# nianticlabs/relpose-gnn

Hardware: AMD Instinct MI355X
Metric: graphs/sec (8-node fully-connected, 224x224) (higher is better)
Workload: dtype f32; 1 GPU; BASELINE.json configs[1]: batch=32 8-node fully-connected graphs per GPU, 224x224 RGB, fp32, ResNet34 + GNN (D=2048, gnn_recursion=2, droprate=0, eval), random-init weights; nodes_per_graph=8, edges_per_graph=56, streams_per_gpu=2, loaded_library=relpose-gnn_amd/lib/librelpose_gnn_hip.so@26afda1856ea

## Files before the change

relpose-gnn_amd/csrc/winograd.hip:

```cpp
#include "rpg_common.h"

typedef float f32x16 __attribute__((ext_vector_type(16)));

namespace {

constexpr int NT = 256;
constexpr int BK = 16, LD = BK;
constexpr int P = 6;
constexpr int BMT = 64, BN = 64;
constexpr int A_FLOATS = P * BMT * LD, B_FLOATS = P * BN * LD;
constexpr int LDS_BYTES = (A_FLOATS + B_FLOATS) * (int)sizeof(float);

struct Epi {
    const float* scale;
    const float* shift;
    const float* residual;
    float* out;
    int relu;
};

__device__ __forceinline__ float4 f4zero() { return make_float4(0.f, 0.f, 0.f, 0.f); }
__device__ __forceinline__ float4 lin(float a, const float4& x, float b, const float4& y) {
    return make_float4(a * x.x + b * y.x, a * x.y + b * y.y, a * x.z + b * y.z, a * x.w + b * y.w);
}
__device__ __forceinline__ float4 add(const float4& x, const float4& y) {
    return make_float4(x.x + y.x, x.y + y.y, x.z + y.z, x.w + y.w);
}
__device__ __forceinline__ float4 sub(const float4& x, const float4& y) {
    return make_float4(x.x - y.x, x.y - y.y, x.z - y.z, x.w - y.w);
}

typedef unsigned int u32x4 __attribute__((ext_vector_type(4)));
typedef float f32x2 __attribute__((ext_vector_type(2)));
__device__ __forceinline__ void wino43_epilogue(const f32x16 (&acc)[P], float* slab, int lane, int mw0, int nw0, int M,
                                                int Tw, int W, int Cout, const Epi& ep) {
    constexpr int EP = 32 + 4;
    constexpr unsigned OOB = 0x80000000u;
    const int c4 = lane & 7, pr = lane >> 3;
    const int nb = nw0 + 4 * c4;
    const bool n_ok = nb < Cout;
    float4 sc = make_float4(1.f, 1.f, 1.f, 1.f), sh = f4zero();
    if (n_ok && ep.scale) sc = *reinterpret_cast<const float4*>(ep.scale + nb);
    if (n_ok && ep.shift) sh = *reinterpret_cast<const float4*>(ep.shift + nb);

    const int t_first = mw0 / Tw;
    const size_t row0 = (size_t)t_first * W * Cout;
    const __amdgpu_buffer_rsrc_t ro = __builtin_amdgcn_make_buffer_rsrc(ep.out + row0, 0, 0x7fffffff, 0x00020000);
    const __amdgpu_buffer_rsrc_t rr = __builtin_amdgcn_make_buffer_rsrc(
        const_cast<float*>(ep.residual ? ep.residual + row0 : ep.out + row0), 0, 0x7fffffff, 0x00020000);
    const int step_t = 4 / Tw, step_tw = 4 % Tw;
    int mt = mw0 + (pr >> 1);
    int trel = mt / Tw - t_first, tw = mt % Tw;
    unsigned voff[2][8];
#pragma unroll
    for (int it = 0; it < 8; ++it) {
        const int wo = 4 * tw + (pr & 1);
        const bool ok = n_ok && mt < M;
        const unsigned o = 4u * (unsigned)((trel * W + wo) * Cout + nb);
        voff[0][it] = ok && wo < W ? o : OOB;
        voff[1][it] = ok && wo + 2 < W ? o + 8u * (unsigned)Cout : OOB;
        mt += 4;
        trel += step_t;
        tw += step_tw;
        if (tw >= Tw) { tw -= Tw; ++trel; }
    }
    float4 rs[2][8];
    if (ep.residual) {
#pragma unroll
        for (int half = 0; half < 2; ++half)
#pragma unroll
            for (int it = 0; it < 8; ++it)
                rs[half][it] = __builtin_bit_cast(float4, __builtin_amdgcn_raw_buffer_load_b128(rr, voff[half][it], 0, 0));
    } else {
#pragma unroll
        for (int half = 0; half < 2; ++half)
#pragma unroll
            for (int it = 0; it < 8; ++it) rs[half][it] = f4zero();
    }
    const bool relu_on = ep.relu;
    f32x2 y[4][8];
#pragma unroll
    for (int q = 0; q < 8; ++q) {
        const int e = 2 * q;
        const f32x2 m0 = {acc[0][e], acc[0][e + 1]}, m1 = {acc[1][e], acc[1][e + 1]}, m2 = {acc[2][e], acc[2][e + 1]};
        const f32x2 m3 = {acc[3][e], acc[3][e + 1]}, m4 = {acc[4][e], acc[4][e + 1]}, m5 = {acc[5][e], acc[5][e + 1]};
        const f32x2 s12 = m1 + m2, d12 = m1 - m2, s34 = m3 + m4, d34 = m3 - m4;
        const f32x2 u = d34 + d34;
        y[0][q] = (m0 + s12) + s34;
        y[1][q] = d12 + u;
        y[2][q] = s12 + 4.f * s34;
        y[3][q] = (d12 + 4.f * u) + m5;
    }
#pragma unroll
    for (int half = 0; half < 2; ++half) {
#pragma unroll
        for (int q = 0; q < 8; ++q) {
            const int e = 2 * q;
            const int trow = (e & 3) + 8 * (e >> 2) + 4 * (lane >> 5);
            float* sp = slab + (2 * trow) * EP + (lane & 31);
            sp[0] = y[2 * half][q].x;
            sp[EP] = y[2 * half + 1][q].x;
            sp[2 * EP] = y[2 * half][q].y;
            sp[3 * EP] = y[2 * half + 1][q].y;
        }
        __builtin_amdgcn_wave_barrier();
#pragma unroll
        for (int it = 0; it < 8; ++it) {
            const int prow = pr + 8 * it;
            const float4 v = *reinterpret_cast<const float4*>(&slab[prow * EP + 4 * c4]);
            const f32x2 r0 = {rs[half][it].x, rs[half][it].y}, r1 = {rs[half][it].z, rs[half][it].w};
            f32x2 o0 = f32x2{v.x, v.y} * f32x2{sc.x, sc.y} + f32x2{sh.x, sh.y} + r0;
            f32x2 o1 = f32x2{v.z, v.w} * f32x2{sc.z, sc.w} + f32x2{sh.z, sh.w} + r1;
            const float4 yv = rpg::relu4_if(relu_on, make_float4(o0.x, o0.y, o1.x, o1.y));
            __builtin_amdgcn_raw_buffer_store_b128(__builtin_bit_cast(u32x4, yv), ro, voff[half][it], 0, 0);
        }
        __builtin_amdgcn_wave_barrier();
    }
}

template <bool RES, class Mid>
__device__ __forceinline__ void wino43_epilogue_lean_body(const f32x16 (&acc)[P], float* slab, int lane, int mw0, int nw0, int M,
                                                          int Tw, int W, int Cout, const Epi& ep, Mid mid) {
    constexpr int EP = 32 + 4;
    constexpr unsigned OOB = 0x80000000u;
    const int c4 = lane & 7, pr = lane >> 3;
    const int nb = nw0 + 4 * c4;
    const bool n_ok = nb < Cout;
    float4 sc = make_float4(1.f, 1.f, 1.f, 1.f), sh = f4zero();
    if (n_ok && ep.scale) sc = *reinterpret_cast<const float4*>(ep.scale + nb);
    if (n_ok && ep.shift) sh = *reinterpret_cast<const float4*>(ep.shift + nb);
    const int t_first = mw0 / Tw;
    const size_t row0 = (size_t)t_first * W * Cout;
    const __amdgpu_buffer_rsrc_t ro = __builtin_amdgcn_make_buffer_rsrc(ep.out + row0, 0, 0x7fffffff, 0x00020000);
    const __amdgpu_buffer_rsrc_t rr = __builtin_amdgcn_make_buffer_rsrc(
        const_cast<float*>(ep.residual ? ep.residual + row0 : ep.out + row0), 0, 0x7fffffff, 0x00020000);
    const int step_t = 4 / Tw, step_tw = 4 % Tw;
    int mt = mw0 + (pr >> 1);
    int trel = mt / Tw - t_first, tw = mt % Tw;
    unsigned voff[8], ok2 = 0;
#pragma unroll
    for (int it = 0; it < 8; ++it) {
// ... 232 lines not shown
        __syncthreads();
        float4 fa[2][2], fb[2][2];
        auto frag_one = [&](int g, int set, int i) {
            const int kb = (g / 3) * 8, xi = 2 * (g % 3) + (i >> 1);
            if (i & 1) fb[set][i >> 1] = *reinterpret_cast<const float4*>(&Bs[xi * BN * LD + (b_off ^ kb)]);
            else       fa[set][i >> 1] = *reinterpret_cast<const float4*>(&As[xi * BMT * LD + (a_off ^ kb)]);
        };
#pragma unroll
        for (int i = 0; i < 4; ++i) frag_one(0, 0, i);
        __builtin_amdgcn_sched_barrier(0);
#pragma unroll
        for (int g = 0; g < 6; ++g) {
            const int set = g & 1, x0 = 2 * (g % 3);
#pragma unroll
            for (int i = 0; i < 8; ++i) {
                const int j = i & 1, e = i >> 1;
                const float av = e == 0 ? fa[set][j].x : e == 1 ? fa[set][j].y : e == 2 ? fa[set][j].z : fa[set][j].w;
                const float bv = e == 0 ? fb[set][j].x : e == 1 ? fb[set][j].y : e == 2 ? fb[set][j].z : fb[set][j].w;
                acc[x0 + j] = __builtin_amdgcn_mfma_f32_32x32x2f32(av, bv, acc[x0 + j], 0, 0, 0);
                if (i < 4 && g + 1 < 6) frag_one(g + 1, set ^ 1, i);
                if (i >= 4 && i < 6) fetch_one(2 * g + (i - 4));
                __builtin_amdgcn_sched_barrier(0);
            }
        }
        fetch_next();
    }
    __syncthreads();

    const int ws = __builtin_amdgcn_readfirstlane(wave);
    wino43_epilogue(acc, lds + ws * (64 * 36), lane, m0 + (ws >> 1) * 32, n0 + (ws & 1) * 32, M, Tw, W, Cout, ep);
}

constexpr int NT8 = 512, BMT8 = 128;
constexpr int A8_FLOATS = P * BMT8 * LD, IMG8_FLOATS = A8_FLOATS + B_FLOATS;
constexpr int LDS8_BYTES = 2 * IMG8_FLOATS * (int)sizeof(float);

typedef float f32x2 __attribute__((ext_vector_type(2)));
struct F4 { f32x2 lo, hi; };
__device__ __forceinline__ F4 to_f4(const float4& v) { return F4{f32x2{v.x, v.y}, f32x2{v.z, v.w}}; }
__device__ __forceinline__ float4 to_float4(const F4& v) { return make_float4(v.lo.x, v.lo.y, v.hi.x, v.hi.y); }
#define RPG_PK_FMA(NAME, CONST)                                                                               \
    __device__ __forceinline__ f32x2 NAME(f32x2 x, f32x2 y) {                                                 \
        f32x2 r;                                                                                              \
        asm("v_pk_fma_f32 %0, %1, " CONST ", %2 op_sel_hi:[1,0,1]" : "=v"(r) : "v"(x), "v"(y));               \
        return r;                                                                                             \
    }
RPG_PK_FMA(pk_fma_p4, "4.0")
RPG_PK_FMA(pk_fma_m4, "-4.0")
RPG_PK_FMA(pk_fma_p2, "2.0")
RPG_PK_FMA(pk_fma_m2, "-2.0")
#undef RPG_PK_FMA
__device__ __forceinline__ f32x2 pk_add(f32x2 x, f32x2 y) {
    f32x2 r;
    asm("v_pk_add_f32 %0, %1, %2" : "=v"(r) : "v"(x), "v"(y));
    return r;
}
__device__ __forceinline__ f32x2 pk_sub(f32x2 x, f32x2 y) {
    f32x2 r;
    asm("v_pk_add_f32 %0, %1, %2 neg_lo:[0,1] neg_hi:[0,1]" : "=v"(r) : "v"(x), "v"(y));
    return r;
}
#define RPG_F4_OP(NAME, OP) \
    __device__ __forceinline__ F4 NAME(const F4& x, const F4& y) { return F4{OP(x.lo, y.lo), OP(x.hi, y.hi)}; }
RPG_F4_OP(fma4_p4, pk_fma_p4)
RPG_F4_OP(fma4_m4, pk_fma_m4)
RPG_F4_OP(fma4_p2, pk_fma_p2)
RPG_F4_OP(fma4_m2, pk_fma_m2)
RPG_F4_OP(add4, pk_add)
RPG_F4_OP(sub4, pk_sub)
#undef RPG_F4_OP

struct Split { int tile_base, parts, n_split; float* partial; unsigned* arrive; };

#ifdef RPG_WINO_TRACE
__device__ unsigned long long* g_wino_trace = nullptr;
#define RPG_TRACE(i)                                                                         \
    do {                                                                                     \
        if (g_wino_trace && threadIdx.x == 0) g_wino_trace[5 * blockIdx.x + (i)] = __builtin_readcyclecounter(); \
    } while (0)
#else
#define RPG_TRACE(i) do {} while (0)
#endif

__device__ __forceinline__ void wino43_finish_quad(const float4& s, const Epi& ep, int tile, int p, int c4, int M, int Tw, int W,
                                                   int Cout, int tiles_n) {
    const int m = (tile / tiles_n) * BMT8 + (p >> 2), nb = (tile % tiles_n) * BN + 4 * c4;
    if (m >= M || nb >= Cout) return;
    const int t = m / Tw, wo = 4 * (m - t * Tw) + (p & 3);
    if (wo >= W) return;
    const size_t o = ((size_t)t * W + wo) * Cout + nb;
    float4 sc = make_float4(1.f, 1.f, 1.f, 1.f), sh = f4zero(), rs = f4zero();
    if (ep.scale) sc = *reinterpret_cast<const float4*>(ep.scale + nb);
    if (ep.shift) sh = *reinterpret_cast<const float4*>(ep.shift + nb);
    if (ep.residual) rs = *reinterpret_cast<const float4*>(ep.residual + o);
    float4 y;
    y.x = s.x * sc.x + sh.x + rs.x; y.y = s.y * sc.y + sh.y + rs.y;
    y.z = s.z * sc.z + sh.z + rs.z; y.w = s.w * sc.w + sh.w + rs.w;
    if (ep.relu) y = rpg::relu4(y);
    *reinterpret_cast<float4*>(ep.out + o) = y;
}

__device__ __forceinline__ void wino43_combine_last(const Split& sp, int tt, const Epi& ep, int M, int Tw, int W, int Cout,
                                                    int tiles_n, int* flag) {
    if (!rpg::last_arriver(sp.arrive + tt, (unsigned)sp.parts, flag)) return;
    const __amdgpu_buffer_rsrc_t rs = rpg::agent_rsrc(sp.partial + (size_t)tt * sp.parts * (BMT8 * 4 * BN));
    constexpr unsigned SLAB_B = BMT8 * 4 * BN * 4;
    const int tile = sp.tile_base + tt;
    const int tid_c = threadIdx.x;
#pragma unroll 1
    for (int h = 0; h < 2; ++h) {
        const unsigned vo = 16u * (unsigned)(tid_c + h * 8 * NT8);
        float4 sum[8];
#pragma unroll
        for (int c = 0; c < 8; ++c) sum[c] = rpg::agent_load_f4(rs, vo + 16u * c * NT8, 0);
        for (int i = 1; i < sp.parts; ++i) {
            float4 v[8];
#pragma unroll
            for (int c = 0; c < 8; ++c) v[c] = rpg::agent_load_f4(rs, vo + 16u * c * NT8, (unsigned)i * SLAB_B);
#pragma unroll
            for (int c = 0; c < 8; ++c) { sum[c].x += v[c].x; sum[c].y += v[c].y; sum[c].z += v[c].z; sum[c].w += v[c].w; }
        }
#pragma unroll
        for (int c = 0; c < 8; ++c) {
            const int idx = tid_c + NT8 * (8 * h + c);
            wino43_finish_quad(sum[c], ep, tile, idx >> 4, idx & 15, M, Tw, W, Cout, tiles_n);
        }
    }
}

__global__ __launch_bounds__(NT8) void wino43_conv8_kernel(const float* __restrict__ x, const float* __restrict__ U, int H,
                                                          int W, int Cin, int Cout, int Tw, int M, Epi ep, int tiles_n,
                                                          Split sp) {
    extern __shared__ __attribute__((aligned(16))) float lds[];
#ifdef RPG_WINO_TRACE
    if (g_wino_trace && threadIdx.x == 0) g_wino_trace[5 * blockIdx.x] = __builtin_amdgcn_s_getreg(0xF804);
#endif
    RPG_TRACE(1);
    const int K = 3 * Cin;
    const int kpr = (Cin + BK - 1) / BK;
    int tile, kb = 0, nk = 3 * kpr;
    const bool is_split = (int)blockIdx.x < sp.n_split;
    if (is_split) {
        const int tt = blockIdx.x / sp.parts, part = blockIdx.x - tt * sp.parts;
        tile = sp.tile_base + tt;
        kb = 3 * (part * kpr / sp.parts);
        nk = 3 * ((part + 1) * kpr / sp.parts);
    } else {
        const int nwg = gridDim.x - sp.n_split, bid = blockIdx.x - sp.n_split;
        const int xcd = bid & 7, loc = bid >> 3, q = nwg >> 3, r8 = nwg & 7;
        tile = (xcd < r8 ? xcd * (q + 1) : r8 * (q + 1) + (xcd - r8) * q) + loc;
    }
    const int m0 = (tile / tiles_n) * BMT8;
    const int n0 = (tile % tiles_n) * BN;

    const int tid = threadIdx.x, lane = tid & 63, wave = tid >> 6;
    const int wm = wave >> 1, wn = wave & 1;
    const int row = tid >> 2, slot = tid & 3;
    const int brow = row & 63, bhalf = tid >> 8;

    const int n_first = (m0 / Tw) / H;
    const size_t img_floats = (size_t)H * W * Cin;
    const __amdgpu_buffer_rsrc_t ra = __builtin_amdgcn_make_buffer_rsrc(
        const_cast<float*>(x + n_first * img_floats) - (size_t)W * Cin, 0, 0x7fffffff, 0x00020000);
    const __amdgpu_buffer_rsrc_t rb = __builtin_amdgcn_make_buffer_rsrc(const_cast<float*>(U), 0, 0x7fffffff, 0x00020000);
    constexpr unsigned OOB = 0x80000000u;
    unsigned va[P], va3[3][P];
    unsigned rowbits = 0;
    {
        const int m = m0 + row;
        int img_off = 0, ho = 0, wi0 = -(1 << 24);
        if (m < M) {
            const int tw = m % Tw;
            const int t = m / Tw;
            ho = t % H;
            img_off = (t / H - n_first) * (int)img_floats;
            wi0 = 4 * tw - 1;
            rowbits = (ho > 0 ? 1u : 0u) | 2u | (ho < H - 1 ? 4u : 0u);
        }
#pragma unroll
        for (int j = 0; j < P; ++j) {
            const int wi = wi0 + j;
            va[j] = (unsigned)wi < (unsigned)W ? 4u * (unsigned)(img_off + (ho * W + wi) * Cin + 4 * slot) : OOB;
        }
    }
    const unsigned ustride_b = (unsigned)Cout * K * 4u;
    const unsigned vb = n0 + brow < Cout ? 4u * (unsigned)((n0 + brow) * K + 4 * slot) + 3u * bhalf * ustride_b : OOB;
    unsigned vb_eff;
    int f_kt = kb, f_c0 = (kb / 3) * BK;
    const unsigned row_b = 4u * (unsigned)(W * Cin), krow_b = 4u * (unsigned)Cin;
    auto refresh = [&]() {
        asm volatile("" ::: "memory");
        const bool cv = f_kt < nk && f_c0 + 4 * slot < Cin;
#pragma unroll
        for (int kh = 0; kh < 3; ++kh) {
            const bool rv = cv && ((rowbits >> kh) & 1u);
#pragma unroll
            for (int j = 0; j < P; ++j) va3[kh][j] = rv ? va[j] : OOB;
        }
        vb_eff = cv ? vb : OOB;
    };
    refresh();

    float4 d[P], ub[3];
    auto fetch_one = [&](int i, int kh) {
        if (i < P) {
            const unsigned sa = (unsigned)kh * row_b + 4u * (unsigned)f_c0;
            d[i] = __builtin_bit_cast(float4, __builtin_amdgcn_raw_buffer_load_b128(ra, va3[kh][i], sa, 0));
        } else {
            const unsigned sb = (unsigned)kh * krow_b + 4u * (unsigned)f_c0 + (unsigned)(i - P) * ustride_b;
            ub[i - P] = __builtin_bit_cast(float4, __builtin_amdgcn_raw_buffer_load_b128(rb, vb_eff, sb, 0));
        }
    };
    auto fetch_next = [&](int kh) {
        ++f_kt;
        if (kh == 2) {
            f_c0 += BK;
            if (f_c0 + BK > Cin || f_kt >= nk) refresh();
        }
    };

    const int st_a = row * LD + 4 * (slot ^ ((row >> 2) & 3));
    const int st_b = A8_FLOATS + (3 * bhalf) * BN * LD + brow * LD + 4 * (slot ^ ((brow >> 2) & 3));
    auto stage_one = [&](int p, int img) {
        if (p >= P) {
            *reinterpret_cast<float4*>(lds + img + st_b + (p - P) * BN * LD) = ub[p - P];
            return;
        }
        const F4 d0 = to_f4(d[0]), d1 = to_f4(d[1]), d2 = to_f4(d[2]), d3 = to_f4(d[3]), d4 = to_f4(d[4]), d5 = to_f4(d[5]);
        F4 v;
        if (p == 0) v = fma4_p4(sub4(d0, d2), sub4(d4, d2));
        else if (p == 5) v = fma4_m4(sub4(d3, d1), sub4(d5, d3));
        else if (p <= 2) {
            const F4 sx = fma4_m4(d2, d4);
            const F4 tx = fma4_m4(d1, d3);
            v = p == 1 ? add4(sx, tx) : sub4(sx, tx);
        } else {
            const F4 r = sub4(d4, d2), t = sub4(d3, d1);
            v = p == 3 ? fma4_p2(t, r) : fma4_m2(t, r);
        }
        *reinterpret_cast<float4*>(lds + img + st_a + p * BMT8 * LD) = to_float4(v);
    };

    f32x16 acc[P];
#pragma unroll
    for (int xi = 0; xi < P; ++xi)
#pragma unroll
        for (int e = 0; e < 16; ++e) acc[xi][e] = 0.f;

    const int rsw = 4 * ((lane >> 5) ^ ((lane >> 2) & 3));
    const int a_off = (wm * 32 + (lane & 31)) * LD + rsw;
    const int b_off = A8_FLOATS + (wn * 32 + (lane & 31)) * LD + rsw;
    float4 fa[2][2], fb[2][2];
    auto frag_one = [&](int g, int set, int i, int img) {
        const int kb = (g / 3) * 8, xi = 2 * (g % 3) + (i >> 1);
        if (i & 1) fb[set][i >> 1] = *reinterpret_cast<const float4*>(&lds[img + xi * BN * LD + (b_off ^ kb)]);
        else       fa[set][i >> 1] = *reinterpret_cast<const float4*>(&lds[img + xi * BMT8 * LD + (a_off ^ kb)]);
    };
    auto kstep = [&](int cur, int nxt, int khf) {
        __builtin_amdgcn_sched_barrier(0);
#pragma unroll
        for (int g = 0; g < 6; ++g) {
            const int set = g & 1, x0 = 2 * (g % 3);
#pragma unroll
            for (int i = 0; i < 8; ++i) {
                const int j = i & 1, e = i >> 1;
                const float av = e == 0 ? fa[set][j].x : e == 1 ? fa[set][j].y : e == 2 ? fa[set][j].z : fa[set][j].w;
                const float bv = e == 0 ? fb[set][j].x : e == 1 ? fb[set][j].y : e == 2 ? fb[set][j].z : fb[set][j].w;
                acc[x0 + j] = __builtin_amdgcn_mfma_f32_32x32x2f32(av, bv, acc[x0 + j], 0, 0, 0);
                if (i < 4) {
                    if (g < 5) frag_one(g + 1, set ^ 1, i, cur);
                    else frag_one(0, 0, i, nxt);
                } else {
                    const int s = 4 * (g % 3) + (i - 4);
                    if (s < 9) {
                        if (g < 3) stage_one(s, nxt);
                        else fetch_one(s, khf);
                    }
                }
                __builtin_amdgcn_sched_barrier(0);
            }
            if (g == 4) {
                __syncthreads();
                __builtin_amdgcn_sched_barrier(0);
            }
        }
        fetch_next(khf);
    };

#pragma unroll
    for (int i = 0; i < 9; ++i) fetch_one(i, 0);
    fetch_next(0);
#pragma unroll
    for (int p = 0; p < 9; ++p) stage_one(p, 0);
#pragma unroll
    for (int i = 0; i < 9; ++i) fetch_one(i, 1);
    fetch_next(1);
    __syncthreads();
#pragma unroll
    for (int i = 0; i < 4; ++i) frag_one(0, 0, i, 0);
    RPG_TRACE(2);
    int kt = kb;
    for (; kt + 5 < nk; kt += 6) {
        kstep(0, IMG8_FLOATS, 2);
        kstep(IMG8_FLOATS, 0, 0);
        kstep(0, IMG8_FLOATS, 1);
        kstep(IMG8_FLOATS, 0, 2);
        kstep(0, IMG8_FLOATS, 0);
        kstep(IMG8_FLOATS, 0, 1);
    }
    if (kt < nk) {
        kstep(0, IMG8_FLOATS, 2);
        kstep(IMG8_FLOATS, 0, 0);
        kstep(0, IMG8_FLOATS, 1);
    }
    __syncthreads();
    RPG_TRACE(3);
    const int ws = __builtin_amdgcn_readfirstlane(wave);
    if (is_split) {
        wino43_epilogue_partial(acc, lds + ws * (64 * 36), lane, (ws >> 1) * 32, (ws & 1) * 32,
                                sp.partial + (size_t)blockIdx.x * (BMT8 * 4 * BN));
        if (sp.arrive) wino43_combine_last(sp, tile - sp.tile_base, ep, M, Tw, W, Cout, tiles_n, reinterpret_cast<int*>(lds));
    } else
        wino43_epilogue(acc, lds + ws * (64 * 36), lane, m0 + (ws >> 1) * 32, n0 + (ws & 1) * 32, M, Tw, W, Cout, ep);
#ifdef RPG_WINO_TRACE
    asm volatile("s_waitcnt vmcnt(0)" ::: "memory");
#endif
    RPG_TRACE(4);
}

__global__ __launch_bounds__(NT8) void wino43_conv8p_kernel(const float* __restrict__ x, const float* __restrict__ U, int H,
                                                           int W, int Cin, int Cout, int Tw, int M, Epi ep, int tiles_n,
                                                           Split sp, int n_items) {
    extern __shared__ __attribute__((aligned(16))) float lds[];
#ifdef RPG_ABL_STAGGER
    {
        const unsigned long long t0 = __builtin_readcyclecounter();
        const unsigned long long wait = (unsigned long long)((blockIdx.x >> 3) & 7) * RPG_ABL_STAGGER;
        while (__builtin_readcyclecounter() - t0 < wait) __builtin_amdgcn_s_sleep(8);
    }
#endif
    const int K = 3 * Cin;
    const int kpr = Cin / BK;
    const int tid = threadIdx.x, lane = tid & 63, wave = tid >> 6;
    const int wm = wave >> 1, wn = wave & 1;
    const int row = tid >> 2, slot = tid & 3;
    const int brow = row & 63, bhalf = tid >> 8;
    const size_t img_floats = (size_t)H * W * Cin;
    const __amdgpu_buffer_rsrc_t rb = __builtin_amdgcn_make_buffer_rsrc(const_cast<float*>(U), 0, 0x7fffffff, 0x00020000);
    constexpr unsigned OOB = 0x80000000u;
    const unsigned ustride_b = (unsigned)Cout * K * 4u;
    const unsigned row_b = 4u * (unsigned)(W * Cin), krow_b = 4u * (unsigned)Cin;

    int f_item = blockIdx.x, f_m0 = 0, f_n0 = 0, f_kb = 0, f_nk = 0, f_kt = 0, f_c0 = 0;
    const float* f_base = x;
    unsigned va3[3][P], vb_eff;
    auto decode = [&]() {
        asm volatile("" ::: "memory");
        int tid_d = tid;
        asm volatile("" : "+v"(tid_d));
        const int row = tid_d >> 2, slot = tid_d & 3, brow = row & 63, bhalf = tid_d >> 8;
        const bool valid = f_item < n_items;
        int tile, kb = 0, nk = 3 * kpr;
        if (f_item < sp.n_split) {
            const int tt = f_item / sp.parts, part = f_item - tt * sp.parts;
            tile = sp.tile_base + tt;
            kb = 3 * (part * kpr / sp.parts);
            nk = 3 * ((part + 1) * kpr / sp.parts);
        } else {
            const int nwg = n_items - sp.n_split, bid = f_item - sp.n_split;
            const int xcd = bid & 7, loc = bid >> 3, q = nwg >> 3, r8 = nwg & 7;
            tile = (xcd < r8 ? xcd * (q + 1) : r8 * (q + 1) + (xcd - r8) * q) + loc;
        }
        f_m0 = (tile / tiles_n) * BMT8;
        f_n0 = (tile - (tile / tiles_n) * tiles_n) * BN;
        const int n_first = (f_m0 / Tw) / H;
        f_base = x + n_first * img_floats - (size_t)W * Cin;
        const int m = f_m0 + row;
        int img_off = 0, ho = 0, wi0 = -(1 << 24);
        unsigned rowbits = 0;
        if (valid && m < M) {
            const int t = m / Tw;
            const int tw = m - t * Tw;
            const int n = t / H;
            ho = t - n * H;
            img_off = (n - n_first) * (int)img_floats;
            wi0 = 4 * tw - 1;
            rowbits = (ho > 0 ? 1u : 0u) | 2u | (ho < H - 1 ? 4u : 0u);
        }
#pragma unroll
        for (int j = 0; j < P; ++j) {
            const int wi = wi0 + j;
            const unsigned o = (unsigned)wi < (unsigned)W ? 4u * (unsigned)(img_off + (ho * W + wi) * Cin + 4 * slot) : OOB;
            va3[0][j] = (rowbits & 1u) ? o : OOB;
            va3[1][j] = OOB;
            va3[2][j] = (rowbits & 4u) ? o : OOB;
        }
        vb_eff = valid && f_n0 + brow < Cout ? 4u * (unsigned)((f_n0 + brow) * K + 4 * slot) + 3u * bhalf * ustride_b : OOB;
        f_kb = kb;
        f_kt = kb;
        f_nk = valid ? nk : 0x3fffffff;
        f_c0 = (kb / 3) * BK;
    };
    auto fix_row1 = [&]() {
#pragma unroll
        for (int j = 0; j < P; ++j) va3[1][j] = va3[0][j] < va3[2][j] ? va3[0][j] : va3[2][j];
    };
// ... 91 lines not shown
#ifndef RPG_ABL_NOBAR
            if (g == 4) {
                __syncthreads();
                __builtin_amdgcn_sched_barrier(0);
            }
#endif
        }
        fetch_next(khf);
    };

    int c_item = f_item, c_m0 = f_m0, c_n0 = f_n0, c_ns = f_nk - f_kb;
#pragma unroll
    for (int i = 0; i < 9; ++i) fetch_one(i, 0);
    fetch_next(0);
#pragma unroll
    for (int p = 0; p < 9; ++p) stage_one(p, X);
#pragma unroll
    for (int i = 0; i < 9; ++i) fetch_one(i, 1);
    fetch_next(1);
    const int ws = __builtin_amdgcn_readfirstlane(wave);
    for (;;) {
#ifdef RPG_WINO_TRACE
        if (g_wino_trace && threadIdx.x == 0) {
            g_wino_trace[5 * c_item] = __builtin_amdgcn_s_getreg(0xF804);
            g_wino_trace[5 * c_item + 1] = __builtin_readcyclecounter();
        }
#endif
#pragma unroll
        for (int xi = 0; xi < P; ++xi)
#pragma unroll
            for (int e = 0; e < 16; ++e) acc[xi][e] = 0.f;
        __syncthreads();
#pragma unroll
        for (int i = 0; i < 4; ++i) frag_one(0, 0, i, X);
#ifdef RPG_WINO_TRACE
        if (g_wino_trace && threadIdx.x == 0) g_wino_trace[5 * c_item + 2] = __builtin_readcyclecounter();
#endif
        int s = 0;
        for (; s + 6 <= c_ns; s += 6) {
            kstep(X, Y, 2);
            kstep(Y, X, 0);
            kstep(X, Y, 1);
            kstep(Y, X, 2);
            kstep(X, Y, 0);
            kstep(Y, X, 1);
        }
        if (s < c_ns) {
            kstep(X, Y, 2);
            kstep(Y, X, 0);
            kstep(X, Y, 1);
            const Img t = X;
            X = Y;
            Y = t;
            ybase = IMG8_FLOATS - ybase;
        }
        __syncthreads();
        float* slab = lds + ybase + ws * (64 * 36);
#ifdef RPG_WINO_TRACE
        if (g_wino_trace && threadIdx.x == 0) g_wino_trace[5 * c_item + 3] = __builtin_readcyclecounter();
#endif
        auto refetch = [&]() {
            fix_row1();
#pragma unroll
            for (int i = 0; i < 9; ++i) fetch_one(i, 1);
        };
        int lane_e = lane;
        asm volatile("" : "+v"(lane_e));
        if (c_item < sp.n_split)
            wino43_epilogue_partial(acc, slab, lane_e, (ws >> 1) * 32, (ws & 1) * 32,
                                    sp.partial + (size_t)c_item * (BMT8 * 4 * BN), refetch);
        else
            wino43_epilogue_lean(acc, slab, lane_e, c_m0 + (ws >> 1) * 32, c_n0 + (ws & 1) * 32, M, Tw, W, Cout, ep, refetch);
#ifdef RPG_WINO_TRACE
        if (g_wino_trace && threadIdx.x == 0) g_wino_trace[5 * c_item + 4] = __builtin_readcyclecounter();
#endif
        if (f_item >= n_items) break;
        c_item = f_item;
        c_m0 = f_m0;
        c_n0 = f_n0;
        c_ns = f_nk - f_kb;
    }
}

__global__ __launch_bounds__(256) void wino43_fixup_kernel(const float* __restrict__ partial, Epi ep, int M, int Tw, int W,
                                                           int Cout, int tiles_n, Split sp) {
    const int tt = blockIdx.x >> 5, idx = (blockIdx.x & 31) * 256 + threadIdx.x;
    const float* src = partial + (size_t)tt * sp.parts * (BMT8 * 4 * BN) + 4 * idx;
    float4 s = *reinterpret_cast<const float4*>(src);
    for (int i = 1; i < sp.parts; ++i) {
        const float4 v = *reinterpret_cast<const float4*>(src + (size_t)i * (BMT8 * 4 * BN));
        s.x += v.x; s.y += v.y; s.z += v.z; s.w += v.w;
    }
    wino43_finish_quad(s, ep, sp.tile_base + tt, idx >> 4, idx & 15, M, Tw, W, Cout, tiles_n);
}

__global__ __launch_bounds__(NT) void wino43_weights_kernel(const float* __restrict__ w, float* __restrict__ U, int Cout,
                                                            int Cin, long total) {
    const long i = (long)blockIdx.x * NT + threadIdx.x;
    if (i >= total) return;
    const int c = (int)(i % Cin);
    const long t = i / Cin;
    const int kh = (int)(t % 3);
    const long co = t / 3;
    const float* wp = w + ((co * 3 + kh) * 3) * (long)Cin + c;
    const double g0 = wp[0], g1 = wp[Cin], g2 = wp[2 * (long)Cin];
    const double u[6] = {g0 / 4.0, -(g0 + g1 + g2) / 6.0, -(g0 - g1 + g2) / 6.0,
                         g0 / 24.0 + g1 / 12.0 + g2 / 6.0, g0 / 24.0 - g1 / 12.0 + g2 / 6.0, g2};
    const long plane = (long)Cout * 3 * Cin;
#pragma unroll
    for (int xi = 0; xi < 6; ++xi) U[xi * plane + i] = (float)u[xi];
}


}

#ifdef RPG_PROBE_WINO2D
#include "../../tools/probes/winograd2d.hip"
#endif

namespace rpg {

bool wino_pays(int n, int h, int w, int cin, int cout) {
    if (!tuning().wino.on || (cin & 3) || (cout & 3)) return false;
    const long tiles = (long)n * h * ((w + 3) / 4);
    const long blocks = ((tiles + BMT - 1) / BMT) * ((cout + BN - 1) / BN);
    const int tw = (w + 3) / 4;
    return blocks >= tuning().wino.min_blocks && (long)h * w * cin * 4 * 67 < (1L << 31) && 6L * cout * 3 * cin * 4 < (1L << 31) &&
           (32L / tw + 3) * w * cout * 4 < (1L << 31);
}

int launch_conv_wino(const float* x, const float* u, const float* scale, const float* shift, const float* residual,
                     float* y, int n, int h, int w, int cin, int cout, int relu, hipStream_t s) {
    if (!x || !u || !y || n <= 0 || h <= 0 || w <= 0 || cin <= 0 || cout <= 0 || (cin & 3) || (cout & 3) ||
        !aligned16(x) || !aligned16(u) || !aligned16(y) || (scale && !aligned16(scale)) || (shift && !aligned16(shift)) ||
        (residual && !aligned16(residual)))
        return RPG_ERR_BAD_ARG;
#ifdef RPG_PROBE_WINO2D
    if (wino2d_takes(n, h, w, cin, cout))
        return launch_conv_wino2d(x, u + (size_t)18 * cout * cin, scale, shift, residual, y, n, h, w, cin, cout, relu, s);
#endif
    const int tw = (w + 3) / 4;
    const long M = (long)n * h * tw;
    if (M >= (1L << 31) || (long)h * w * cin * 4 * 67 >= (1L << 31) || 6L * cout * 3 * cin * 4 >= (1L << 31) ||
        (32L / tw + 3) * w * cout * 4 >= (1L << 31))
        return RPG_ERR_BAD_ARG;
    int dev = 0;
    if (hipGetDevice(&dev) != hipSuccess || dev < 0 || dev >= 64) dev = 0;
    static bool attr[64] = {};
    if (!attr[dev]) {
        (void)hipFuncSetAttribute(reinterpret_cast<const void*>(wino43_conv_kernel),
                                  hipFuncAttributeMaxDynamicSharedMemorySize, LDS_BYTES);
        attr[dev] = true;
    }
    const int tn = (cout + BN - 1) / BN;
    Epi ep{scale, shift, residual, y, relu};
    const int slot = timing_begin(RPG_TIMER_CONV_WINO, s);
    double executed = 0.0;
    const long tm8 = (M + BMT8 - 1) / BMT8;
    const bool fits8 = (long)h * w * cin * 4 * 131 < (1L << 31);
    if (fits8 && (tuning().wino.on == 3 || (tuning().wino.on == 1 && tm8 * tn >= 8))) {
        static bool attr8[64] = {};
        if (!attr8[dev]) {
            (void)hipFuncSetAttribute(reinterpret_cast<const void*>(wino43_conv8_kernel),
                                      hipFuncAttributeMaxDynamicSharedMemorySize, LDS8_BYTES);
            attr8[dev] = true;
        }
        const long T = tm8 * tn;
        const int S = num_cus(), kpr = (cin + BK - 1) / BK, nk = 3 * kpr;
        executed = (double)T * nk * 48.0 * 8.0 * 4096.0;
        long t_main = T;
        Split sp{0, 1, 0, nullptr, nullptr};
        const long tail = T % S;
        if (tuning().wino.persist && cin % BK == 0 && (T > S || tuning().wino.persist == 2) && h >= 2) {
            static bool attr8p[64] = {};
            if (!attr8p[dev]) {
                (void)hipFuncSetAttribute(reinterpret_cast<const void*>(wino43_conv8p_kernel),
                                          hipFuncAttributeMaxDynamicSharedMemorySize, LDS8_BYTES);
                attr8p[dev] = true;
            }
            if (tuning().wino.split && tail > 0) {
                int parts = (int)(S / tail);
                if (parts > kpr) parts = kpr;
                if (parts >= 2) {
                    sp.partial = stream_scratch(s, (size_t)tail * parts * (BMT8 * 4 * BN) * sizeof(float));
                    if (sp.partial) { sp.parts = parts; t_main = T - tail; sp.tile_base = (int)t_main; sp.n_split = (int)(tail * parts); }
                }
            }
            const long items = sp.n_split + t_main;
            hipLaunchKernelGGL(wino43_conv8p_kernel, dim3((unsigned)(items < S ? items : S)), dim3(NT8), LDS8_BYTES, s, x, u, h, w,
                               cin, cout, tw, (int)M, ep, tn, sp, (int)items);
            if (sp.n_split) {
                hipStream_t fs = fixup_hop_begin(s);
                hipLaunchKernelGGL(wino43_fixup_kernel, dim3((unsigned)(T - t_main) * 32), dim3(256), 0, fs, sp.partial, ep, (int)M,
                                   tw, w, cout, tn, sp);
                fixup_hop_end(s, fs);
            }
            timing_end(slot, 2.0 * (double)n * h * w * cout * 9.0 * cin, s, executed);
            RPG_CHECK_LAUNCH("conv3x3_wino43");
            return RPG_OK;
        }
        if (tuning().wino.split && tail > 0) {
            int parts = (int)(S / tail);
            if (parts > kpr) parts = kpr;
            if (parts > nk / tuning().wino.split_steps && nk / tuning().wino.split_steps >= 2) parts = nk / tuning().wino.split_steps;
            if (parts >= 2) {
                unsigned* counters = nullptr;
                sp.partial = stream_scratch(s, (size_t)tail * parts * (BMT8 * 4 * BN) * sizeof(float), &counters);
                if (sp.partial) { sp.parts = parts; t_main = T - tail; sp.tile_base = (int)t_main; sp.n_split = (int)(tail * parts); }
                if (sp.partial && (tuning().gemm.inkernel_fixup & 2) && parts <= tuning().wino.combine_max) sp.arrive = counters;
            }
        }
        hipLaunchKernelGGL(wino43_conv8_kernel, dim3((unsigned)(sp.n_split + t_main)), dim3(NT8), LDS8_BYTES, s, x, u, h, w, cin,
                           cout, tw, (int)M, ep, tn, sp);
        if (sp.n_split && !sp.arrive) {
            hipStream_t fs = fixup_hop_begin(s);
            hipLaunchKernelGGL(wino43_fixup_kernel, dim3((unsigned)(T - t_main) * 32), dim3(256), 0, fs, sp.partial, ep, (int)M, tw, w,
                               cout, tn, sp);
            fixup_hop_end(s, fs);
        }
    } else {
        const int tm = (int)((M + BMT - 1) / BMT);
        executed = (double)tm * tn * (3 * ((cin + BK - 1) / BK)) * 48.0 * 4.0 * 4096.0;
        hipLaunchKernelGGL(wino43_conv_kernel, dim3(tm * tn), dim3(NT), LDS_BYTES, s, x, u, h, w, cin, cout, tw, (int)M, ep, tn);
    }
    timing_end(slot, 2.0 * (double)n * h * w * cout * 9.0 * cin, s, executed);
    RPG_CHECK_LAUNCH("conv3x3_wino43");
    return RPG_OK;
}

}

#ifdef RPG_WINO_TRACE
extern "C" int rpg_wino_trace_set(unsigned long long* buf) {
    return hipMemcpyToSymbol(HIP_SYMBOL(g_wino_trace), &buf, sizeof(buf)) == hipSuccess ? RPG_OK : RPG_ERR_LAUNCH;
}
#endif

extern "C" size_t rpg_wino43_weights_floats(int cout, int cin) {
    if (cout <= 0 || cin <= 0) return 0;
#ifdef RPG_PROBE_WINO2D
    return rpg::wino_weight_floats(cout, cin);
#else
    return (size_t)18 * cout * cin;
#endif
}

extern "C" int rpg_wino43_transform_weights_f32(const float* w_ohwi, float* u, int cout, int cin, void* stream) {
    if (!w_ohwi || !u || cout <= 0 || cin <= 0) return RPG_ERR_BAD_ARG;
    const long total = (long)cout * 3 * cin;
    hipLaunchKernelGGL(wino43_weights_kernel, dim3((unsigned)((total + NT - 1) / NT)), dim3(NT), 0, rpg::as_stream(stream),
                       w_ohwi, u, cout, cin, total);
    RPG_CHECK_LAUNCH("wino43_transform_weights");
#ifdef RPG_PROBE_WINO2D
    return rpg::launch_wino2d_weights(w_ohwi, u + (size_t)18 * cout * cin, cout, cin, rpg::as_stream(stream));
#else
    return RPG_OK;
#endif
}

extern "C" int rpg_conv3x3_wino43_bn_act_nhwc_f32(const float* x, const float* u, const float* scale, const float* shift,
                                                  const float* residual, float* y, int n, int h, int w, int cin, int cout,
                                                  int relu, void* stream) {
    return rpg::launch_conv_wino(x, u, scale, shift, residual, y, n, h, w, cin, cout, relu, rpg::as_stream(stream));
}
```

Measured before the change: 3093 graphs/s.

## Add row-major tile ordering to Winograd conv8 to skip padded kernel rows

```diff
diff --git a/relpose-gnn_amd/csrc/winograd.hip b/relpose-gnn_amd/csrc/winograd.hip
--- a/relpose-gnn_amd/csrc/winograd.hip
+++ b/relpose-gnn_amd/csrc/winograd.hip
@@ -32,8 +32,31 @@
 
 typedef unsigned int u32x4 __attribute__((ext_vector_type(4)));
 typedef float f32x2 __attribute__((ext_vector_type(2)));
+
+struct RowOrder { int H, ntw; };
+template <bool RM>
+__device__ __forceinline__ int wino43_block_m0(int j, const RowOrder& ro) {
+    if constexpr (RM) {
+        const int col = j / ro.H, ho = j - col * ro.H;
+        return ho * ro.ntw + col * 128;
+    } else
+        return j * 128;
+}
+template <bool RM>
+__device__ __forceinline__ void wino43_tile_row(int m, int Tw, const RowOrder& ro, int& t, int& tw) {
+    if constexpr (RM) {
+        const int ho = m / ro.ntw, i = m - ho * ro.ntw, img = i / Tw;
+        t = img * ro.H + ho;
+        tw = i - img * Tw;
+    } else {
+        t = m / Tw;
+        tw = m - t * Tw;
+    }
+}
+
+template <bool RM = false>
 __device__ __forceinline__ void wino43_epilogue(const f32x16 (&acc)[P], float* slab, int lane, int mw0, int nw0, int M,
-                                                int Tw, int W, int Cout, const Epi& ep) {
+                                                int Tw, int W, int Cout, const Epi& ep, const RowOrder& ord = RowOrder{0, 0}) {
     constexpr int EP = 32 + 4;
     constexpr unsigned OOB = 0x80000000u;
     const int c4 = lane & 7, pr = lane >> 3;
@@ -43,20 +66,27 @@
     if (n_ok && ep.scale) sc = *reinterpret_cast<const float4*>(ep.scale + nb);
     if (n_ok && ep.shift) sh = *reinterpret_cast<const float4*>(ep.shift + nb);
 
-    const int t_first = mw0 / Tw;
+    int i0 = mw0, t_scale = 1, t_add = 0, row_px = W;
+    if constexpr (RM) {
+        t_add = mw0 / ord.ntw;
+        i0 = mw0 - t_add * ord.ntw;
+        t_scale = ord.H;
+        row_px = ord.H * W;
+    }
+    const int q_first = i0 / Tw, t_first = q_first * t_scale + t_add;
     const size_t row0 = (size_t)t_first * W * Cout;
     const __amdgpu_buffer_rsrc_t ro = __builtin_amdgcn_make_buffer_rsrc(ep.out + row0, 0, 0x7fffffff, 0x00020000);
     const __amdgpu_buffer_rsrc_t rr = __builtin_amdgcn_make_buffer_rsrc(
         const_cast<float*>(ep.residual ? ep.residual + row0 : ep.out + row0), 0, 0x7fffffff, 0x00020000);
     const int step_t = 4 / Tw, step_tw = 4 % Tw;
     int mt = mw0 + (pr >> 1);
-    int trel = mt / Tw - t_first, tw = mt % Tw;
+    int trel = (i0 + (pr >> 1)) / Tw - q_first, tw = (i0 + (pr >> 1)) % Tw;
     unsigned voff[2][8];
 #pragma unroll
     for (int it = 0; it < 8; ++it) {
         const int wo = 4 * tw + (pr & 1);
         const bool ok = n_ok && mt < M;
-        const unsigned o = 4u * (unsigned)((trel * W + wo) * Cout + nb);
+        const unsigned o = 4u * (unsigned)((trel * row_px + wo) * Cout + nb);
         voff[0][it] = ok && wo < W ? o : OOB;
         voff[1][it] = ok && wo + 2 < W ? o + 8u * (unsigned)Cout : OOB;
         mt += 4;
@@ -455,11 +485,14 @@
 #define RPG_TRACE(i) do {} while (0)
 #endif
 
+template <bool RM>
 __device__ __forceinline__ void wino43_finish_quad(const float4& s, const Epi& ep, int tile, int p, int c4, int M, int Tw, int W,
-                                                   int Cout, int tiles_n) {
-    const int m = (tile / tiles_n) * BMT8 + (p >> 2), nb = (tile % tiles_n) * BN + 4 * c4;
+                                                   int Cout, int tiles_n, const RowOrder& ord) {
+    const int m = wino43_block_m0<RM>(tile / tiles_n, ord) + (p >> 2), nb = (tile % tiles_n) * BN + 4 * c4;
     if (m >= M || nb >= Cout) return;
-    const int t = m / Tw, wo = 4 * (m - t * Tw) + (p & 3);
+    int t, tw;
+    wino43_tile_row<RM>(m, Tw, ord, t, tw);
+    const int wo = 4 * tw + (p & 3);
     if (wo >= W) return;
     const size_t o = ((size_t)t * W + wo) * Cout + nb;
     float4 sc = make_float4(1.f, 1.f, 1.f, 1.f), sh = f4zero(), rs = f4zero();
@@ -473,8 +506,9 @@
     *reinterpret_cast<float4*>(ep.out + o) = y;
 }
 
+template <bool RM>
 __device__ __forceinline__ void wino43_combine_last(const Split& sp, int tt, const Epi& ep, int M, int Tw, int W, int Cout,
-                                                    int tiles_n, int* flag) {
+                                                    int tiles_n, const RowOrder& ord, int* flag) {
     if (!rpg::last_arriver(sp.arrive + tt, (unsigned)sp.parts, flag)) return;
     const __amdgpu_buffer_rsrc_t rs = rpg::agent_rsrc(sp.partial + (size_t)tt * sp.parts * (BMT8 * 4 * BN));
     constexpr unsigned SLAB_B = BMT8 * 4 * BN * 4;
@@ -496,55 +530,68 @@
 #pragma unroll
         for (int c = 0; c < 8; ++c) {
             const int idx = tid_c + NT8 * (8 * h + c);
-            wino43_finish_quad(sum[c], ep, tile, idx >> 4, idx & 15, M, Tw, W, Cout, tiles_n);
-        }
-    }
-}
-
+            wino43_finish_quad<RM>(sum[c], ep, tile, idx >> 4, idx & 15, M, Tw, W, Cout, tiles_n, ord);
+        }
+    }
+}
+
+template <bool RM>
 __global__ __launch_bounds__(NT8) void wino43_conv8_kernel(const float* __restrict__ x, const float* __restrict__ U, int H,
                                                           int W, int Cin, int Cout, int Tw, int M, Epi ep, int tiles_n,
-                                                          Split sp) {
+                                                          Split sp, int ntw) {
     extern __shared__ __attribute__((aligned(16))) float lds[];
 #ifdef RPG_WINO_TRACE
     if (g_wino_trace && threadIdx.x == 0) g_wino_trace[5 * blockIdx.x] = __builtin_amdgcn_s_getreg(0xF804);
 #endif
     RPG_TRACE(1);
     const int K = 3 * Cin;
+    const RowOrder ord{H, ntw};
     const int kpr = (Cin + BK - 1) / BK;
     int tile, kb = 0, nk = 3 * kpr;
+    int cb0 = 0, cb1 = kpr;
     const bool is_split = (int)blockIdx.x < sp.n_split;
     if (is_split) {
         const int tt = blockIdx.x / sp.parts, part = blockIdx.x - tt * sp.parts;
         tile = sp.tile_base + tt;
-        kb = 3 * (part * kpr / sp.parts);
-        nk = 3 * ((part + 1) * kpr / sp.parts);
+        cb0 = part * kpr / sp.parts;
+        cb1 = (part + 1) * kpr / sp.parts;
+        kb = 3 * cb0;
+        nk = 3 * cb1;
     } else {
         const int nwg = gridDim.x - sp.n_split, bid = blockIdx.x - sp.n_split;
         const int xcd = bid & 7, loc = bid >> 3, q = nwg >> 3, r8 = nwg & 7;
         tile = (xcd < r8 ? xcd * (q + 1) : r8 * (q + 1) + (xcd - r8) * q) + loc;
     }
-    const int m0 = (tile / tiles_n) * BMT8;
+    const int m0 = wino43_block_m0<RM>(tile / tiles_n, ord);
     const int n0 = (tile % tiles_n) * BN;
+    int kh0 = 0, kh_end = 3;
+    if constexpr (RM) {
+        const int ho = m0 / ntw;
+        kh0 = ho == 0 ? 1 : 0;
+        kh_end = ho == H - 1 ? 2 : 3;
+        kb = 0;
+        nk = (kh_end - kh0) * (cb1 - cb0);
+    }
 
     const int tid = threadIdx.x, lane = tid & 63, wave = tid >> 6;
     const int wm = wave >> 1, wn = wave & 1;
     const int row = tid >> 2, slot = tid & 3;
     const int brow = row & 63, bhalf = tid >> 8;
 
-    const int n_first = (m0 / Tw) / H;
+    const int n_first = RM ? (m0 % ntw) / Tw : (m0 / Tw) / H;
     const size_t img_floats = (size_t)H * W * Cin;
     const __amdgpu_buffer_rsrc_t ra = __builtin_amdgcn_make_buffer_rsrc(
         const_cast<float*>(x + n_first * img_floats) - (size_t)W * Cin, 0, 0x7fffffff, 0x00020000);
     const __amdgpu_buffer_rsrc_t rb = __builtin_amdgcn_make_buffer_rsrc(const_cast<float*>(U), 0, 0x7fffffff, 0x00020000);
     constexpr unsigned OOB = 0x80000000u;
-    unsigned va[P], va3[3][P];
+    unsigned va[P], va3[RM ? 1 : 3][P];
     unsigned rowbits = 0;
     {
         const int m = m0 + row;
         int img_off = 0, ho = 0, wi0 = -(1 << 24);
         if (m < M) {
-            const int tw = m % Tw;
-            const int t = m / Tw;
+            int t, tw;
+            wino43_tile_row<RM>(m, Tw, ord, t, tw);
             ho = t % H;
             img_off = (t / H - n_first) * (int)img_floats;
             wi0 = 4 * tw - 1;
@@ -559,14 +606,15 @@
     const unsigned ustride_b = (unsigned)Cout * K * 4u;
     const unsigned vb = n0 + brow < Cout ? 4u * (unsigned)((n0 + brow) * K + 4 * slot) + 3u * bhalf * ustride_b : OOB;
     unsigned vb_eff;
-    int f_kt = kb, f_c0 = (kb / 3) * BK;
+    int f_kt = kb, f_c0 = cb0 * BK;
+    int f_kh = kh0;
     const unsigned row_b = 4u * (unsigned)(W * Cin), krow_b = 4u * (unsigned)Cin;
     auto refresh = [&]() {
         asm volatile("" ::: "memory");
         const bool cv = f_kt < nk && f_c0 + 4 * slot < Cin;
 #pragma unroll
-        for (int kh = 0; kh < 3; ++kh) {
-            const bool rv = cv && ((rowbits >> kh) & 1u);
+        for (int kh = 0; kh < (RM ? 1 : 3); ++kh) {
+            const bool rv = cv && (RM || ((rowbits >> kh) & 1u));
 #pragma unroll
             for (int j = 0; j < P; ++j) va3[kh][j] = rv ? va[j] : OOB;
         }
@@ -575,18 +623,24 @@
     refresh();
 
     float4 d[P], ub[3];
-    auto fetch_one = [&](int i, int kh) {
+    auto fetch_one = [&](int i, int kh_c) {
+        const unsigned kh = RM ? (unsigned)f_kh : (unsigned)kh_c;
         if (i < P) {
-            const unsigned sa = (unsigned)kh * row_b + 4u * (unsigned)f_c0;
-            d[i] = __builtin_bit_cast(float4, __builtin_amdgcn_raw_buffer_load_b128(ra, va3[kh][i], sa, 0));
+            const unsigned sa = kh * row_b + 4u * (unsigned)f_c0;
+            d[i] = __builtin_bit_cast(float4, __builtin_amdgcn_raw_buffer_load_b128(ra, va3[RM ? 0 : kh_c][i], sa, 0));
         } else {
-            const unsigned sb = (unsigned)kh * krow_b + 4u * (unsigned)f_c0 + (unsigned)(i - P) * ustride_b;
+            const unsigned sb = kh * krow_b + 4u * (unsigned)f_c0 + (unsigned)(i - P) * ustride_b;
             ub[i - P] = __builtin_bit_cast(float4, __builtin_amdgcn_raw_buffer_load_b128(rb, vb_eff, sb, 0));
         }
     };
     auto fetch_next = [&](int kh) {
         ++f_kt;
-        if (kh == 2) {
+        bool wrap = kh == 2;
+        if constexpr (RM) {
+            wrap = ++f_kh == kh_end;
+            if (wrap) f_kh = kh0;
+        }
+        if (wrap) {
             f_c0 += BK;
             if (f_c0 + BK > Cin || f_kt >= nk) refresh();
         }
@@ -673,18 +727,26 @@
     for (int i = 0; i < 4; ++i) frag_one(0, 0, i, 0);
     RPG_TRACE(2);
     int kt = kb;
-    for (; kt + 5 < nk; kt += 6) {
-        kstep(0, IMG8_FLOATS, 2);
-        kstep(IMG8_FLOATS, 0, 0);
-        kstep(0, IMG8_FLOATS, 1);
-        kstep(IMG8_FLOATS, 0, 2);
-        kstep(0, IMG8_FLOATS, 0);
-        kstep(IMG8_FLOATS, 0, 1);
-    }
-    if (kt < nk) {
-        kstep(0, IMG8_FLOATS, 2);
-        kstep(IMG8_FLOATS, 0, 0);
-        kstep(0, IMG8_FLOATS, 1);
+    if constexpr (RM) {
+        for (; kt + 1 < nk; kt += 2) {
+            kstep(0, IMG8_FLOATS, 0);
+            kstep(IMG8_FLOATS, 0, 0);
+        }
+        if (kt < nk) kstep(0, IMG8_FLOATS, 0);
+    } else {
+        for (; kt + 5 < nk; kt += 6) {
+            kstep(0, IMG8_FLOATS, 2);
+            kstep(IMG8_FLOATS, 0, 0);
+            kstep(0, IMG8_FLOATS, 1);
+            kstep(IMG8_FLOATS, 0, 2);
+            kstep(0, IMG8_FLOATS, 0);
+            kstep(IMG8_FLOATS, 0, 1);
+        }
+        if (kt < nk) {
+            kstep(0, IMG8_FLOATS, 2);
+            kstep(IMG8_FLOATS, 0, 0);
+            kstep(0, IMG8_FLOATS, 1);
+        }
     }
     __syncthreads();
     RPG_TRACE(3);
@@ -692,9 +754,9 @@
     if (is_split) {
         wino43_epilogue_partial(acc, lds + ws * (64 * 36), lane, (ws >> 1) * 32, (ws & 1) * 32,
                                 sp.partial + (size_t)blockIdx.x * (BMT8 * 4 * BN));
-        if (sp.arrive) wino43_combine_last(sp, tile - sp.tile_base, ep, M, Tw, W, Cout, tiles_n, reinterpret_cast<int*>(lds));
+        if (sp.arrive) wino43_combine_last<RM>(sp, tile - sp.tile_base, ep, M, Tw, W, Cout, tiles_n, ord, reinterpret_cast<int*>(lds));
     } else
-        wino43_epilogue(acc, lds + ws * (64 * 36), lane, m0 + (ws >> 1) * 32, n0 + (ws & 1) * 32, M, Tw, W, Cout, ep);
+        wino43_epilogue<RM>(acc, lds + ws * (64 * 36), lane, m0 + (ws >> 1) * 32, n0 + (ws & 1) * 32, M, Tw, W, Cout, ep, ord);
 #ifdef RPG_WINO_TRACE
     asm volatile("s_waitcnt vmcnt(0)" ::: "memory");
 #endif
@@ -952,8 +1014,9 @@
     }
 }
 
+template <bool RM>
 __global__ __launch_bounds__(256) void wino43_fixup_kernel(const float* __restrict__ partial, Epi ep, int M, int Tw, int W,
-                                                           int Cout, int tiles_n, Split sp) {
+                                                           int Cout, int tiles_n, Split sp, RowOrder ord) {
     const int tt = blockIdx.x >> 5, idx = (blockIdx.x & 31) * 256 + threadIdx.x;
     const float* src = partial + (size_t)tt * sp.parts * (BMT8 * 4 * BN) + 4 * idx;
     float4 s = *reinterpret_cast<const float4*>(src);
@@ -961,7 +1024,7 @@
         const float4 v = *reinterpret_cast<const float4*>(src + (size_t)i * (BMT8 * 4 * BN));
         s.x += v.x; s.y += v.y; s.z += v.z; s.w += v.w;
     }
-    wino43_finish_quad(s, ep, sp.tile_base + tt, idx >> 4, idx & 15, M, Tw, W, Cout, tiles_n);
+    wino43_finish_quad<RM>(s, ep, sp.tile_base + tt, idx >> 4, idx & 15, M, Tw, W, Cout, tiles_n, ord);
 }
 
 __global__ __launch_bounds__(NT) void wino43_weights_kernel(const float* __restrict__ w, float* __restrict__ U, int Cout,
@@ -1031,16 +1094,26 @@
     if (fits8 && (tuning().wino.on == 3 || (tuning().wino.on == 1 && tm8 * tn >= 8))) {
         static bool attr8[64] = {};
         if (!attr8[dev]) {
-            (void)hipFuncSetAttribute(reinterpret_cast<const void*>(wino43_conv8_kernel),
+            (void)hipFuncSetAttribute(reinterpret_cast<const void*>(wino43_conv8_kernel<false>),
+                                      hipFuncAttributeMaxDynamicSharedMemorySize, LDS8_BYTES);
+            (void)hipFuncSetAttribute(reinterpret_cast<const void*>(wino43_conv8_kernel<true>),
                                       hipFuncAttributeMaxDynamicSharedMemorySize, LDS8_BYTES);
             attr8[dev] = true;
         }
         const long T = tm8 * tn;
         const int S = num_cus(), kpr = (cin + BK - 1) / BK, nk = 3 * kpr;
-        executed = (double)T * nk * 48.0 * 8.0 * 4096.0;
         long t_main = T;
         Split sp{0, 1, 0, nullptr, nullptr};
         const long tail = T % S;
+        const long ntw = (long)n * tw;
+        const bool rm_fits = ntw % BMT8 == 0 && h >= 2 && (128L / tw + 4) * h * w * cin * 4 < (1L << 31) &&
+                             (32L / tw + 3) * h * w * cout * 4 < (1L << 31);
+        auto rm_split = [&]() { return sp.n_split == 0 || t_main == 0; };
+        auto executed_flop = [&](bool rm) {
+            const double steps = rm ? (double)T / h * kpr * (3.0 * h - 2.0) : (double)T * nk;
+            return steps * 48.0 * 8.0 * 4096.0;
+        };
+        const RowOrder ord{h, (int)ntw};
         if (tuning().wino.persist && cin % BK == 0 && (T > S || tuning().wino.persist == 2) && h >= 2) {
             static bool attr8p[64] = {};
             if (!attr8p[dev]) {
@@ -1061,10 +1134,11 @@
                                cin, cout, tw, (int)M, ep, tn, sp, (int)items);
             if (sp.n_split) {
                 hipStream_t fs = fixup_hop_begin(s);
-                hipLaunchKernelGGL(wino43_fixup_kernel, dim3((unsigned)(T - t_main) * 32), dim3(256), 0, fs, sp.partial, ep, (int)M,
-                                   tw, w, cout, tn, sp);
+                hipLaunchKernelGGL(wino43_fixup_kernel<false>, dim3((unsigned)(T - t_main) * 32), dim3(256), 0, fs, sp.partial, ep,
+                                   (int)M, tw, w, cout, tn, sp, ord);
                 fixup_hop_end(s, fs);
             }
+            executed = executed_flop(false);
             timing_end(slot, 2.0 * (double)n * h * w * cout * 9.0 * cin, s, executed);
             RPG_CHECK_LAUNCH("conv3x3_wino43");
             return RPG_OK;
@@ -1080,14 +1154,25 @@
                 if (sp.partial && (tuning().gemm.inkernel_fixup & 2) && parts <= tuning().wino.combine_max) sp.arrive = counters;
             }
         }
-        hipLaunchKernelGGL(wino43_conv8_kernel, dim3((unsigned)(sp.n_split + t_main)), dim3(NT8), LDS8_BYTES, s, x, u, h, w, cin,
-                           cout, tw, (int)M, ep, tn, sp);
+        const bool rm = rm_fits && rm_split();
+        const dim3 grid((unsigned)(sp.n_split + t_main));
+        if (rm)
+            hipLaunchKernelGGL(wino43_conv8_kernel<true>, grid, dim3(NT8), LDS8_BYTES, s, x, u, h, w, cin, cout, tw, (int)M, ep, tn, sp,
+                               ord.ntw);
+        else
+            hipLaunchKernelGGL(wino43_conv8_kernel<false>, grid, dim3(NT8), LDS8_BYTES, s, x, u, h, w, cin, cout, tw, (int)M, ep, tn, sp,
+                               ord.ntw);
         if (sp.n_split && !sp.arrive) {
             hipStream_t fs = fixup_hop_begin(s);
-            hipLaunchKernelGGL(wino43_fixup_kernel, dim3((unsigned)(T - t_main) * 32), dim3(256), 0, fs, sp.partial, ep, (int)M, tw, w,
-                               cout, tn, sp);
+            if (rm)
+                hipLaunchKernelGGL(wino43_fixup_kernel<true>, dim3((unsigned)(T - t_main) * 32), dim3(256), 0, fs, sp.partial, ep, (int)M,
+                                   tw, w, cout, tn, sp, ord);
+            else
+                hipLaunchKernelGGL(wino43_fixup_kernel<false>, dim3((unsigned)(T - t_main) * 32), dim3(256), 0, fs, sp.partial, ep, (int)M,
+                                   tw, w, cout, tn, sp, ord);
             fixup_hop_end(s, fs);
         }
+        executed = executed_flop(rm);
     } else {
         const int tm = (int)((M + BMT - 1) / BMT);
         executed = (double)tm * tn * (3 * ((cin + BK - 1) / BK)) * 48.0 * 4.0 * 4096.0;
```

Result: faster. 3138 graphs/s, median of 6 (+1.5%).
